# Aceinna/gnss-ins-sim

Hardware: AMD Instinct MI355X
Metric: Monte-Carlo IMU samples integrated/sec (higher is better)
Workload: dtype f64

## Files before the change

### gnss-ins-sim_amd/csrc/ginsim_api.hip

```cpp
#include <hip/hip_runtime.h>
#include <chrono>

#include <cmath>
#include <cstdarg>
#include <cstdio>
#include <cstring>
#include <string>
#include <vector>

#include "ginsim.h"
#include "ginsim_oallan.h"
#include "ginsim_psd.h"
#include "ginsim_lpsd.h"
#include "ginsim_csd.h"
#include "ginsim_loose_all.h"
#include "ginsim_loose_all_cons.h"
#include "allan.hpp"
#include "oallan.hpp"
#include "psd.hpp"
#include "lpsd.hpp"
#include "csd.hpp"
#include "comm.hpp"
#include "launch.hpp"
#include "placed.hpp"

namespace ginsim {

static thread_local std::string g_err;

void set_error(const char* fmt, ...) {
    char buf[512];
    va_list ap;
    va_start(ap, fmt);
    vsnprintf(buf, sizeof(buf), fmt, ap);
    va_end(ap);
    g_err = buf;
}

}

using namespace ginsim;

struct ginsim_ctx {
    int device;
    hipStream_t stream;
    hipEvent_t ev0, ev1;
    std::vector<hipEvent_t> pool;
    void* ws[4] = {nullptr, nullptr, nullptr, nullptr};
    size_t ws_bytes[4] = {0, 0, 0, 0};
    double* allan_host = nullptr;
    size_t allan_host_doubles = 0;
    int max_grid_y = 65535;
    ginsim::Comm* comm = nullptr;
    double* comm_recv = nullptr;
    ginsim_stats* comm_host = nullptr;
    hipEvent_t comm_ev[8] = {};
    bool comm_pending[8] = {};
    ginsim_stats* stat_slots = nullptr;
    hipEvent_t stat_ev[8] = {};
    bool stat_pending[8] = {};
    unsigned long long* selftest = nullptr;
};

static hipError_t scratch(ginsim_ctx* c, int slot, size_t bytes, void** out) {
    if (c->ws_bytes[slot] < bytes) {
        if (c->ws[slot]) {
            hipError_t e = hipStreamSynchronize(c->stream);
            if (e != hipSuccess) return e;
            e = hipFree(c->ws[slot]);
            if (e != hipSuccess) return e;
            c->ws[slot] = nullptr;
            c->ws_bytes[slot] = 0;
        }
        const size_t want = bytes + bytes / 4 + 4096;
        hipError_t e = hipMalloc(&c->ws[slot], want);
        if (e != hipSuccess) return e;
        c->ws_bytes[slot] = want;
    }
    *out = c->ws[slot];
    return hipSuccess;
}

#define HIP_TRY(expr)                                                                         \
    do {                                                                                      \
        hipError_t e_ = (expr);                                                               \
        if (e_ != hipSuccess) {                                                               \
            set_error("%s failed: %s (%s:%d)", #expr, hipGetErrorString(e_), __FILE__, __LINE__); \
            if (e_ == hipErrorOutOfMemory) { (void)hipGetLastError(); return GINSIM_ERR_NOMEM; } \
            return GINSIM_ERR_HIP;                                                            \
        }                                                                                     \
    } while (0)

#define REQUIRE(cond, ...)            \
    do {                              \
        if (!(cond)) {                \
            set_error(__VA_ARGS__);   \
            return GINSIM_ERR_ARG;    \
        }                             \
    } while (0)

struct DevBuf {
    void* p = nullptr;
    ~DevBuf() { if (p) (void)hipFree(p); }
    hipError_t alloc(size_t bytes) { return hipMalloc(&p, bytes ? bytes : 8); }
    template <class T> T* as() const { return reinterpret_cast<T*>(p); }
};

template <class Launch>
static int gather_run(const char* who, ginsim_ctx* c, const void* series, int32_t ncomp, int64_t n, int64_t runs, const int64_t* run_ids,
                      int32_t nsel, double* host_out, Launch launch) {
    REQUIRE(c && series && run_ids && host_out, "%s: NULL argument", who);
    REQUIRE(ncomp >= 1 && n >= 1 && runs >= 1 && nsel >= 1, "%s: bad sizes", who);
    for (int i = 0; i < nsel; ++i)
        REQUIRE(run_ids[i] >= 0 && run_ids[i] < runs, "%s: run id %lld out of range", who, (long long)run_ids[i]);
    HIP_TRY(hipSetDevice(c->device));
    DevBuf ids, out;
    const size_t out_bytes = sizeof(double) * (size_t)nsel * n * ncomp;
    HIP_TRY(ids.alloc(sizeof(int64_t) * nsel));
    HIP_TRY(out.alloc(out_bytes));
    HIP_TRY(hipMemcpyAsync(ids.p, run_ids, sizeof(int64_t) * nsel, hipMemcpyHostToDevice, c->stream));
    HIP_TRY(launch(ids.as<int64_t>(), out.as<double>()));
    HIP_TRY(hipMemcpyAsync(host_out, out.p, out_bytes, hipMemcpyDeviceToHost, c->stream));
    HIP_TRY(hipStreamSynchronize(c->stream));
    return GINSIM_OK;
}

template <class Launch>
static int traj_run(ginsim_ctx* c, TrajView v, size_t body, double* host_out, size_t out_bytes, Launch launch) {
    HIP_TRY(hipSetDevice(c->device));
    void* ws = nullptr;
    HIP_TRY(scratch(c, 2, body + sizeof(int64_t) * (size_t)v.m, &ws));
    if (v.samples) {
        int64_t* d_samples = reinterpret_cast<int64_t*>(reinterpret_cast<char*>(ws) + body);
        HIP_TRY(hipMemcpyAsync(d_samples, v.samples, sizeof(int64_t) * (size_t)v.m, hipMemcpyHostToDevice, c->stream));
        v.samples = d_samples;
    }
    HIP_TRY(launch(v, ws));
    if (out_bytes) HIP_TRY(hipMemcpyAsync(host_out, ws, out_bytes, hipMemcpyDeviceToHost, c->stream));
    HIP_TRY(hipStreamSynchronize(c->stream));
    return GINSIM_OK;
}

struct AllanStep { int k; int mode; };
struct AllanPlan {
    std::vector<int64_t> mult;
    int levels = 0;
    std::vector<AllanLevel> lvs;
    AllanFold fold;
    int64_t records = 0;
    std::vector<AllanStep> steps;
    std::vector<int32_t> mode, chunks_per_block, nparts;
};

static int allan_factors(int64_t n, double fs, std::vector<int64_t>& mult, int64_t* mmax_out) {
    const double ts = 1.0 / fs;
    const int64_t mmax = *mmax_out = (int64_t)floor((double)n / 9.0);
    if ((double)mmax * ts < 1.0) return 0;
    const int decades = (int)ceil(log10((double)mmax));
    double scale = 0.1;
    for (int i = 0; i < decades; ++i) {
        scale *= 10;
        for (int j = 1; j < 10; ++j) {
            const int64_t m = (int64_t)(j * scale);
            if (m > mmax) break;
            mult.push_back(m);
        }
    }
    return decades;
}

static int allan_plan(const double* x, int64_t n, int32_t nseries, int64_t series_stride, double fs, AllanPlan& P) {
    REQUIRE(n >= 1 && nseries >= 1 && series_stride >= n && fs > 0, "allan: bad sizes");
    int64_t mmax = 0;
    const int decades = allan_factors(n, fs, P.mult, &mmax);
    if ((double)mmax * (1.0 / fs) < 1.0) return GINSIM_OK;
    const int levels = P.levels = decades;
    std::vector<AllanLevel>& lvs = P.lvs;
    lvs.resize(levels);
    AllanFold& fold = P.fold;
    fold.nlevels = 0;
    fold.fused_level = -1;
    fold.pad = 0;
    for (int j = 0; j < 9; ++j) fold.fused_nb[j] = 0;
    int64_t& records = P.records;
    std::vector<AllanStep>& steps = P.steps;
    P.mode.assign(levels, 4);
    P.chunks_per_block.assign(levels, 1);
    P.nparts.assign(levels, 1);
    {
        int64_t n_in = n, stride_in = series_stride, pow10 = 1;
        for (int k = 0; k < levels; ++k) {
            AllanLevel& lv = lvs[k];
            lv.n_in = n_in;
            lv.n_out = (k + 1 < levels) ? n_in / 10 : 0;
            lv.in_stride = stride_in;
            lv.out_stride = lv.n_out;
            for (int j = 1; j <= 9; ++j) lv.nb[j - 1] = (j * pow10 <= mmax) ? n / (j * pow10) : 0;
            lv.nchunks = allan_chunks(n_in);
            lv.chunks_per_block = allan_chunks_per_block((int64_t)lv.nchunks * nseries);
            stride_in = lv.n_out;
            n_in = lv.n_out;
            pow10 *= 10;
        }
        int k = 0;
        if (levels >= 2 && lvs[0].n_in > allan_chunk_entries() && allan_fuse_applies(x, lvs[0], lvs[1])) {
            const int parts = allan_fuse_parts(lvs[0]);
            fold.nparts[0] = parts;
            fold.offset[0] = records;
            records += (int64_t)parts * nseries;
            fold.nparts[1] = parts;
            fold.offset[1] = records;
// ... 703 lines not shown
        REQUIRE(!L.scale_truth || L.scale, "loose_all_cons_run: scale_truth without a scale block");
    }
    if (L.cons && L.cons->cons_m == 0) L.cons = nullptr;
    if (L.mag && L.mag->mag_every == 0) L.mag = nullptr;
    if (L.still && L.still->still_mask == 0) L.still = nullptr;
    L.all_cons = who == LOOSE_ALL_CONS && L.cons != nullptr;
    L.all = (who == LOOSE_ALL || who == LOOSE_ALL_CONS) && (L.mag != nullptr) + (L.scale != nullptr) + (L.still != nullptr) >= 2;
    if (L.name) {
        L.name[0] = 0;
        (void)launch_loose(L);
        return GINSIM_OK;
    }
    HIP_TRY(hipSetDevice(c->device));
    const ginsim_loose_params* p = L.b;
    const size_t sb = sizeof(int64_t) * (size_t)p->m, vb = (sizeof(int32_t) * (size_t)p->m + 7) / 8 * 8;
    const size_t cb = L.cons ? sizeof(int64_t) * (size_t)L.cons->cons_m : 0;
    if (sb + cb > 0) {
        void* ws = nullptr;
        HIP_TRY(scratch(c, 3, sb + vb + cb, &ws));
        if (p->m > 0) {
            int64_t* d_stamp = reinterpret_cast<int64_t*>(ws);
            HIP_TRY(hipMemcpyAsync(d_stamp, p->gps_stamp, sb, hipMemcpyHostToDevice, c->stream));
            L.stamp = d_stamp;
            if (p->gps_visible) {
                int32_t* d_vis = reinterpret_cast<int32_t*>(reinterpret_cast<char*>(ws) + sb);
                HIP_TRY(hipMemcpyAsync(d_vis, p->gps_visible, sizeof(int32_t) * (size_t)p->m, hipMemcpyHostToDevice, c->stream));
                L.visible = d_vis;
            }
        }
        if (cb > 0) {
            int64_t* d_cons = reinterpret_cast<int64_t*>(reinterpret_cast<char*>(ws) + sb + vb);
            HIP_TRY(hipMemcpyAsync(d_cons, L.cons->cons_sample, cb, hipMemcpyHostToDevice, c->stream));
            L.samples = d_cons;
        }
    }
    L.stream = c->stream;
    HIP_TRY(launch_loose(L));
    return GINSIM_OK;
}

int ginsim_loose_kernel_name(const ginsim_mc_params* mc, const ginsim_loose_params* p, char* buf, size_t cap) {
    REQUIRE(buf && cap > 0, "loose_kernel_name: bad arguments");
    return loose_entry(LOOSE_PLAIN, nullptr, LooseLaunch{mc, p, nullptr, nullptr, nullptr, nullptr, buf, cap});
}

int ginsim_loose_run(ginsim_ctx* c, const ginsim_mc_params* mc, const ginsim_loose_params* p) {
    REQUIRE(c, "loose_run: NULL argument");
    return loose_entry(LOOSE_PLAIN, c, LooseLaunch{mc, p});
}

int ginsim_loose_cons_kernel_name(const ginsim_mc_params* mc, const ginsim_loose_params* p, const ginsim_loose_cons_params* cons,
                                  char* buf, size_t cap) {
    REQUIRE(buf && cap > 0, "loose_cons_kernel_name: bad arguments");
    return loose_entry(LOOSE_CONS, nullptr, LooseLaunch{mc, p, cons, nullptr, nullptr, nullptr, buf, cap});
}

int ginsim_loose_cons_run(ginsim_ctx* c, const ginsim_mc_params* mc, const ginsim_loose_params* p, const ginsim_loose_cons_params* cons) {
    REQUIRE(c, "loose_cons_run: NULL argument");
    return loose_entry(LOOSE_CONS, c, LooseLaunch{mc, p, cons});
}

int ginsim_loose_mag_kernel_name(const ginsim_mc_params* mc, const ginsim_loose_params* p, const ginsim_loose_mag_params* mag,
                                 char* buf, size_t cap) {
    REQUIRE(buf && cap > 0, "loose_mag_kernel_name: bad arguments");
    return loose_entry(LOOSE_MAG, nullptr, LooseLaunch{mc, p, nullptr, mag, nullptr, nullptr, buf, cap});
}

int ginsim_loose_mag_run(ginsim_ctx* c, const ginsim_mc_params* mc, const ginsim_loose_params* p, const ginsim_loose_mag_params* mag) {
    REQUIRE(c, "loose_mag_run: NULL argument");
    return loose_entry(LOOSE_MAG, c, LooseLaunch{mc, p, nullptr, mag});
}

int ginsim_loose_scale_kernel_name(const ginsim_mc_params* mc, const ginsim_loose_params* p, const ginsim_loose_scale_params* scale,
                                   char* buf, size_t cap) {
    REQUIRE(buf && cap > 0, "loose_scale_kernel_name: bad arguments");
    return loose_entry(LOOSE_SCALE, nullptr, LooseLaunch{mc, p, nullptr, nullptr, scale, nullptr, buf, cap});
}

int ginsim_loose_scale_run(ginsim_ctx* c, const ginsim_mc_params* mc, const ginsim_loose_params* p, const ginsim_loose_scale_params* scale) {
    REQUIRE(c, "loose_scale_run: NULL argument");
    return loose_entry(LOOSE_SCALE, c, LooseLaunch{mc, p, nullptr, nullptr, scale});
}

int ginsim_loose_still_kernel_name(const ginsim_mc_params* mc, const ginsim_loose_params* p, const ginsim_loose_still_params* still,
                                   char* buf, size_t cap) {
    REQUIRE(buf && cap > 0, "loose_still_kernel_name: bad arguments");
    return loose_entry(LOOSE_STILL, nullptr, LooseLaunch{mc, p, nullptr, nullptr, nullptr, still, buf, cap});
}

int ginsim_loose_still_run(ginsim_ctx* c, const ginsim_mc_params* mc, const ginsim_loose_params* p, const ginsim_loose_still_params* still) {
    REQUIRE(c, "loose_still_run: NULL argument");
    return loose_entry(LOOSE_STILL, c, LooseLaunch{mc, p, nullptr, nullptr, nullptr, still});
}

int ginsim_loose_all_kernel_name(const ginsim_mc_params* mc, const ginsim_loose_params* p, const ginsim_loose_mag_params* mag,
                                 const ginsim_loose_scale_params* scale, const ginsim_loose_still_params* still, char* buf, size_t cap) {
    REQUIRE(buf && cap > 0, "loose_all_kernel_name: bad arguments");
    return loose_entry(LOOSE_ALL, nullptr, LooseLaunch{mc, p, nullptr, mag, scale, still, buf, cap});
}

int ginsim_loose_all_run(ginsim_ctx* c, const ginsim_mc_params* mc, const ginsim_loose_params* p, const ginsim_loose_mag_params* mag,
                         const ginsim_loose_scale_params* scale, const ginsim_loose_still_params* still) {
    REQUIRE(c, "loose_all_run: NULL argument");
    return loose_entry(LOOSE_ALL, c, LooseLaunch{mc, p, nullptr, mag, scale, still});
}

int ginsim_loose_all_cons_kernel_name(const ginsim_mc_params* mc, const ginsim_loose_params* p, const ginsim_loose_mag_params* mag,
                                      const ginsim_loose_scale_params* scale, const ginsim_loose_still_params* still,
                                      const ginsim_loose_cons_params* cons, const double* scale_truth, char* buf, size_t cap) {
    REQUIRE(buf && cap > 0, "loose_all_cons_kernel_name: bad arguments");
    LooseLaunch L{mc, p, cons, mag, scale, still, buf, cap};
    L.scale_truth = scale_truth;
    return loose_entry(LOOSE_ALL_CONS, nullptr, L);
}

int ginsim_loose_all_cons_run(ginsim_ctx* c, const ginsim_mc_params* mc, const ginsim_loose_params* p, const ginsim_loose_mag_params* mag,
                              const ginsim_loose_scale_params* scale, const ginsim_loose_still_params* still,
                              const ginsim_loose_cons_params* cons, const double* scale_truth) {
    REQUIRE(c, "loose_all_cons_run: NULL argument");
    LooseLaunch L{mc, p, cons, mag, scale, still};
    L.scale_truth = scale_truth;
    return loose_entry(LOOSE_ALL_CONS, c, L);
}

int ginsim_aux_sensors(ginsim_ctx* c, const ginsim_aux_params* p) {
    REQUIRE(c && p, "aux_sensors: NULL argument");
    REQUIRE(p->runs >= 1 && p->n >= 0 && p->m >= 0, "aux_sensors: bad sizes");
    REQUIRE(!p->out_gps || p->ref_gps, "aux_sensors: ref_gps missing");
    REQUIRE(!p->out_mag || p->ref_mag, "aux_sensors: ref_mag missing");
    REQUIRE(p->n <= 0xFFFFFFFFll && p->m <= 0xFFFFFFFFll, "aux_sensors: sample index exceeds the RNG counter");
    REQUIRE((double)p->n * (double)p->runs < 5.0e11 && (double)p->m * (double)p->runs < 5.0e11, "aux_sensors: too many elements");
    HIP_TRY(hipSetDevice(c->device));
    HIP_TRY(launch_aux(*p, c->stream));
    return GINSIM_OK;
}

int ginsim_magcal_run(ginsim_ctx* c, const ginsim_magcal_params* p) {
    REQUIRE(c && p, "magcal_run: NULL argument");
    REQUIRE(p->runs >= 1, "magcal_run: runs=%lld must be >= 1", (long long)p->runs);
    REQUIRE(p->n >= 1 && p->n <= 0xFFFFFFFFll, "magcal_run: n must lie in 1 .. the 32-bit sample counter of the RNG");
    REQUIRE(p->runs <= (int64_t)0x7FFFFFFF * 64, "magcal_run: too many runs for one launch");
    REQUIRE(p->in_mag || p->ref_mag, "magcal_run: neither ref_mag (generated form) nor in_mag (given form)");
    REQUIRE(p->out_si && p->out_hi, "magcal_run: out_si / out_hi missing");
    for (int a = 0; a < 3; ++a) {
        const long long s0 = (long long)p->seg[2 * a], s1 = (long long)p->seg[2 * a + 1];
        REQUIRE(s0 >= 0 && s1 <= (long long)p->n, "magcal_run: range %c [%lld, %lld) is outside [0, %lld]", "xyz"[a], s0, s1, (long long)p->n);
        REQUIRE(s0 < s1, "magcal_run: range %c [%lld, %lld) is empty", "xyz"[a], s0, s1);
    }
    HIP_TRY(hipSetDevice(c->device));
    HIP_TRY(launch_magcal(*p, c->stream));
    return GINSIM_OK;
}

int ginsim_end_stats(ginsim_ctx* c, const double* end_err, int64_t runs, ginsim_stats* host_out) {
    REQUIRE(c && end_err && host_out && runs >= 1, "end_stats: bad arguments");
    HIP_TRY(hipSetDevice(c->device));
    void* ws = nullptr;
    HIP_TRY(scratch(c, 0, stats_scratch_bytes(runs), &ws));
    HIP_TRY(launch_end_stats(end_err, runs, ws, c->stream));
    const char* res = reinterpret_cast<char*>(ws) + stats_scratch_bytes(runs) - sizeof(ginsim_stats);
    HIP_TRY(hipMemcpyAsync(host_out, res, sizeof(ginsim_stats), hipMemcpyDeviceToHost, c->stream));
    HIP_TRY(hipStreamSynchronize(c->stream));
    return GINSIM_OK;
}

int ginsim_end_stats_begin(ginsim_ctx* c, const double* end_err, int64_t runs, int32_t slot) {
    REQUIRE(c && end_err && runs >= 1 && slot >= 0 && slot < 8, "end_stats_begin: bad arguments");
    REQUIRE(!c->stat_pending[slot], "end_stats_begin: slot %d is still pending (call ginsim_end_stats_finish first)", slot);
    HIP_TRY(hipSetDevice(c->device));
    if (!c->stat_slots) HIP_TRY(hipHostMalloc(reinterpret_cast<void**>(&c->stat_slots), 8 * sizeof(ginsim_stats), hipHostMallocDefault));
    if (!c->stat_ev[slot]) HIP_TRY(hipEventCreateWithFlags(&c->stat_ev[slot], hipEventDisableTiming));
    void* ws = nullptr;
    HIP_TRY(scratch(c, 0, stats_scratch_bytes(runs), &ws));
    HIP_TRY(launch_end_stats(end_err, runs, ws, c->stream));
    const char* res = reinterpret_cast<char*>(ws) + stats_scratch_bytes(runs) - sizeof(ginsim_stats);
    HIP_TRY(hipMemcpyAsync(&c->stat_slots[slot], res, sizeof(ginsim_stats), hipMemcpyDeviceToHost, c->stream));
    HIP_TRY(hipEventRecord(c->stat_ev[slot], c->stream));
    c->stat_pending[slot] = true;
    return GINSIM_OK;
}

int ginsim_end_stats_finish(ginsim_ctx* c, int32_t slot, ginsim_stats* host_out) {
    REQUIRE(c && host_out && slot >= 0 && slot < 8, "end_stats_finish: bad arguments");
    REQUIRE(c->stat_pending[slot], "end_stats_finish: nothing was begun in slot %d", slot);
    HIP_TRY(hipEventSynchronize(c->stat_ev[slot]));
    *host_out = c->stat_slots[slot];
    c->stat_pending[slot] = false;
    return GINSIM_OK;
}

int ginsim_comm_unique_id(unsigned char* id) {
    REQUIRE(id, "comm_unique_id: NULL output");
    const char* err = comm_unique_id(id);
    if (err) { set_error("comm_unique_id: %s", err); return GINSIM_ERR_HIP; }
    return GINSIM_OK;
}

int ginsim_comm_init(ginsim_ctx* c, int32_t nranks, int32_t rank, const unsigned char* id) {
    REQUIRE(c && id && nranks >= 1 && rank >= 0 && rank < nranks, "comm_init: bad arguments");
    REQUIRE(!c->comm, "comm_init: this context already has a communicator");
    HIP_TRY(hipSetDevice(c->device));
    const size_t bytes = sizeof(ginsim_stats) * 8 * (size_t)nranks;
    hipError_t e = hipMalloc(reinterpret_cast<void**>(&c->comm_recv), bytes);
    if (e == hipSuccess) e = hipHostMalloc(reinterpret_cast<void**>(&c->comm_host), bytes, hipHostMallocDefault);
    const char* err = e == hipSuccess ? comm_create(nranks, rank, id, &c->comm) : nullptr;
    if (e != hipSuccess || err) {
        if (c->comm_recv) { (void)hipFree(c->comm_recv); c->comm_recv = nullptr; }
        if (c->comm_host) { (void)hipHostFree(c->comm_host); c->comm_host = nullptr; }
        c->comm = nullptr;
        if (err) set_error("comm_init: %s", err);
        else set_error("comm_init: %s", hipGetErrorString(e));
        return GINSIM_ERR_HIP;
    }
    return GINSIM_OK;
}

int ginsim_comm_probe(void) {
    const char* err = comm_probe();
    if (err) { set_error("comm_probe: %s", err); return GINSIM_ERR_HIP; }
    return GINSIM_OK;
}

__global__ void first_xcc_kernel(uint32_t* out) {
    if (threadIdx.x == 0) out[0] = __builtin_amdgcn_s_getreg((31 << 11) | 20) & 0xf;
}

int ginsim_stream_first_xcc(ginsim_ctx* c, int32_t* xcc) {
    REQUIRE(c && xcc, "stream_first_xcc: NULL argument");
    HIP_TRY(hipSetDevice(c->device));
    void* ws = nullptr;
    HIP_TRY(scratch(c, 2, 64, &ws));
    hipLaunchKernelGGL(first_xcc_kernel, dim3(1), dim3(64), 0, c->stream, reinterpret_cast<uint32_t*>(ws));
    HIP_TRY(hipGetLastError());
    uint32_t v = 0;
    HIP_TRY(hipMemcpyAsync(&v, ws, sizeof v, hipMemcpyDeviceToHost, c->stream));
    HIP_TRY(hipStreamSynchronize(c->stream));
    *xcc = (int32_t)v;
    return GINSIM_OK;
}

int ginsim_vib_psd_series(ginsim_ctx* c, const double* amp, int64_t period, int64_t runs, uint64_t run_offset, uint64_t seed,
                          int32_t sensor, int32_t halve_per_run, double* out) {
    REQUIRE(c && amp && out, "vib_psd_series: NULL argument");
    REQUIRE(period >= 2 && period <= 16384 && period % 2 == 0, "vib_psd_series: period %lld must be even, 2 .. 16384 (time_series_from_psd.py:36-43)",
            (long long)period);
    REQUIRE(runs >= 1 && runs <= (int64_t)0x7FFFFFFF * 64, "vib_psd_series: runs=%lld out of range", (long long)runs);
    REQUIRE(sensor == 0 || sensor == 1, "vib_psd_series: sensor must be 0 (accelerometer) or 1 (gyroscope)");
    REQUIRE(halve_per_run == 0 || halve_per_run == 1, "vib_psd_series: halve_per_run must be 0 or 1");
    for (int64_t k = 0; k < 3 * (period / 2 + 1); ++k)
        REQUIRE(std::isfinite(amp[k]) && amp[k] >= 0.0, "vib_psd_series: amplitude %lld is negative or not finite", (long long)k);
    HIP_TRY(hipSetDevice(c->device));
    void* ws = nullptr;
    HIP_TRY(scratch(c, 3, vib_psd_scratch_bytes(period, runs), &ws));
    return launch_vib_psd(c->device, c->stream, amp, period, runs, run_offset, seed, sensor, halve_per_run, ws, out);
}

int ginsim_comm_query(ginsim_ctx* c, int32_t* nranks, int32_t* rank, int32_t* device) {
    REQUIRE(c && nranks && rank && device, "comm_query: bad arguments");
    REQUIRE(c->comm, "comm_query: no communicator (ginsim_comm_init)");
    int n = -1, r = -1, d = -1;
    const char* err = comm_query(c->comm, &n, &r, &d);
    if (err) { set_error("comm_query: %s", err); return GINSIM_ERR_HIP; }
    *nranks = n; *rank = r; *device = d;
    return GINSIM_OK;
}

int ginsim_comm_destroy(ginsim_ctx* c) {
    REQUIRE(c, "comm_destroy: NULL context");
    if (!c->comm) return GINSIM_OK;
    HIP_TRY(hipSetDevice(c->device));
    HIP_TRY(hipStreamSynchronize(c->stream));
    comm_destroy(c->comm);
    c->comm = nullptr;
    if (c->comm_recv) { (void)hipFree(c->comm_recv); c->comm_recv = nullptr; }
    if (c->comm_host) { (void)hipHostFree(c->comm_host); c->comm_host = nullptr; }
    for (bool& p : c->comm_pending) p = false;
    return GINSIM_OK;
}

int ginsim_end_stats_all_begin(ginsim_ctx* c, const double* end_err, int64_t runs, int32_t slot) {
    REQUIRE(c && runs >= 0 && (runs == 0 || end_err) && slot >= 0 && slot < 8, "end_stats_all_begin: bad arguments");
    REQUIRE(c->comm && c->comm_recv && c->comm_host, "end_stats_all_begin: no communicator (ginsim_comm_init)");
    REQUIRE(!c->comm_pending[slot], "end_stats_all_begin: slot %d is still pending (call ginsim_end_stats_all_finish first)", slot);
    HIP_TRY(hipSetDevice(c->device));
    if (!c->comm_ev[slot]) HIP_TRY(hipEventCreateWithFlags(&c->comm_ev[slot], hipEventDisableTiming));
    const int nranks = comm_nranks(c->comm);
    void* ws = nullptr;
    const size_t wb = stats_scratch_bytes(runs > 0 ? runs : 1);
    HIP_TRY(scratch(c, 0, wb, &ws));
    double* rec = reinterpret_cast<double*>(reinterpret_cast<char*>(ws) + wb - sizeof(ginsim_stats));
    if (runs > 0) HIP_TRY(launch_end_stats(end_err, runs, ws, c->stream));
    else HIP_TRY(hipMemsetAsync(rec, 0, sizeof(ginsim_stats), c->stream));
    double* recv = c->comm_recv + (size_t)slot * nranks * (sizeof(ginsim_stats) / sizeof(double));
    const char* err = comm_allgather_f64(c->comm, rec, recv, sizeof(ginsim_stats) / sizeof(double), c->stream);
    if (err) { set_error("end_stats_all_begin: %s", err); return GINSIM_ERR_HIP; }
    HIP_TRY(hipMemcpyAsync(c->comm_host + (size_t)slot * nranks, recv, sizeof(ginsim_stats) * nranks, hipMemcpyDeviceToHost, c->stream));
    HIP_TRY(hipEventRecord(c->comm_ev[slot], c->stream));
    c->comm_pending[slot] = true;
    return GINSIM_OK;
}

int ginsim_end_stats_all_finish(ginsim_ctx* c, int32_t slot, ginsim_stats* merged) {
    REQUIRE(c && merged && slot >= 0 && slot < 8, "end_stats_all_finish: bad arguments");
    REQUIRE(c->comm && c->comm_pending[slot], "end_stats_all_finish: nothing was begun in slot %d", slot);
    HIP_TRY(hipEventSynchronize(c->comm_ev[slot]));
    c->comm_pending[slot] = false;
    const int nranks = comm_nranks(c->comm);
    std::vector<ginsim_stats> parts;
    for (int r = 0; r < nranks; ++r) {
        const ginsim_stats& p = c->comm_host[(size_t)slot * nranks + r];
        if (p.count > 0) parts.push_back(p);
    }
    memset(merged, 0, sizeof(*merged));
    if (!parts.empty()) stats_merge_host(parts.data(), (int)parts.size(), merged);
    return GINSIM_OK;
}

static int traj_stats_run(ginsim_ctx* c, const TrajView& v, int64_t first_sample, int32_t pos_ned, double* proc_out, ginsim_stats* end_out) {
    HIP_TRY(hipSetDevice(c->device));
    void* ws = nullptr;
    const size_t bytes = sizeof(double) * 27 * (size_t)v.runs;
    HIP_TRY(scratch(c, 2, bytes, &ws));
    double* rec = reinterpret_cast<double*>(ws);
    HIP_TRY(launch_process_stats(v, proc_out ? first_sample : v.n - 1, pos_ned, proc_out ? 1 : 0, rec, c->stream));
    if (!proc_out) return ginsim_end_stats(c, rec + (size_t)9 * v.runs, v.runs, end_out);
    HIP_TRY(hipMemcpyAsync(proc_out, ws, bytes, hipMemcpyDeviceToHost, c->stream));
    HIP_TRY(hipStreamSynchronize(c->stream));
    return GINSIM_OK;
}

int ginsim_process_stats(ginsim_ctx* c, const double* traj, const double* ref, int64_t n, int64_t runs, int64_t first_sample,
                         int32_t pos_ned, double* host_out) {
    REQUIRE(c && traj && ref && host_out, "process_stats: NULL argument");
    REQUIRE(n >= 1 && runs >= 1 && first_sample >= 0 && first_sample < n, "process_stats: bad sizes");
    return traj_stats_run(c, TrajView{traj, 0, ref, n, runs, nullptr, 0, {nullptr, 0, 0}}, first_sample, pos_ned, host_out, nullptr);
}

int ginsim_end_stats_from_traj(ginsim_ctx* c, const double* traj, const double* ref, int64_t n, int64_t runs, int32_t pos_ned,
                               ginsim_stats* host_out) {
    REQUIRE(c && traj && ref && host_out && n >= 1 && runs >= 1, "end_stats_from_traj: bad arguments");
    return traj_stats_run(c, TrajView{traj, 0, ref, n, runs, nullptr, 0, {nullptr, 0, 0}}, 0, pos_ned, nullptr, host_out);
}

int ginsim_process_stats_f32(ginsim_ctx* c, const float* traj, const double* ref, int64_t n, int64_t runs, int64_t first_sample,
                             int32_t pos_ned, const double* origin, int32_t n_ini, uint64_t ini_first, double* host_out) {
    REQUIRE(c && traj && ref && origin && host_out, "process_stats_f32: NULL argument");
    REQUIRE(n >= 1 && runs >= 1 && first_sample >= 0 && first_sample < n && n_ini >= 1, "process_stats_f32: bad sizes");
    return traj_stats_run(c, TrajView{traj, 1, ref, n, runs, nullptr, 0, {origin, n_ini, ini_first}}, first_sample, pos_ned, host_out, nullptr);
}

int ginsim_end_stats_from_traj_f32(ginsim_ctx* c, const float* traj, const double* ref, int64_t n, int64_t runs, int32_t pos_ned,
                                   const double* origin, int32_t n_ini, uint64_t ini_first, ginsim_stats* host_out) {
    REQUIRE(c && traj && ref && origin && host_out && n >= 1 && runs >= 1 && n_ini >= 1, "end_stats_from_traj_f32: bad arguments");
    return traj_stats_run(c, TrajView{traj, 1, ref, n, runs, nullptr, 0, {origin, n_ini, ini_first}}, 0, pos_ned, nullptr, host_out);
}

static int check_curve_args(const char* who, const void* c, const TrajView& v, const void* host_out) {
    const int64_t n = v.n, m = v.m;
    REQUIRE(c && v.traj && v.ref && host_out, "%s: NULL argument", who);
    REQUIRE(n >= 1 && v.runs >= 1, "%s: n=%lld runs=%lld must be >= 1", who, (long long)n, (long long)v.runs);
    REQUIRE(m >= 1, "%s: m=%lld samples (at least one is needed)", who, (long long)m);
    REQUIRE(v.samples || m == n, "%s: samples == NULL means every sample, so m must be n (m=%lld, n=%lld)", who, (long long)m, (long long)n);
    REQUIRE(m <= 0x7FFFFFFFll, "%s: too many samples for one call", who);
    if (v.samples)
        for (int64_t i = 0; i < m; ++i)
            REQUIRE(v.samples[i] >= 0 && v.samples[i] < n, "%s: sample %lld (entry %lld) is outside [0, %lld)", who, (long long)v.samples[i],
                    (long long)i, (long long)n);
    return GINSIM_OK;
}

static int check_which(const char* who, int32_t which) {
    REQUIRE(which == 0 || which == 1, "%s: which=%d is neither 0 (position) nor 1 (velocity)", who, (int)which);
    return GINSIM_OK;
}

static int check_origin(const char* who, const TrajView& v) {
    REQUIRE(!v.f32 || (v.org.table && v.org.n_ini >= 1), "%s: the origin table of the displacement series is missing", who);
    return GINSIM_OK;
}

static int curve_entry(const char* who, ginsim_ctx* c, const TrajView& v, int32_t pos_ned, double* host_out) {
    int rc = check_curve_args(who, c, v, host_out);
    if (!rc) rc = check_origin(who, v);
    if (rc) return rc;
    return traj_run(c, v, error_curve_scratch_bytes(v), host_out, sizeof(double) * 36 * (size_t)v.m,
                    [&](const TrajView& d, void* ws) { return launch_error_curve(d, pos_ned, ws, c->stream); });
}

int ginsim_error_curve(ginsim_ctx* c, const double* traj, const double* ref, int64_t n, int64_t runs, const int64_t* samples, int64_t m,
                       int32_t pos_ned, double* host_out) {
    return curve_entry("error_curve", c, TrajView{traj, 0, ref, n, runs, samples, m, {nullptr, 0, 0}}, pos_ned, host_out);
}

int ginsim_error_curve_f32(ginsim_ctx* c, const float* traj, const double* ref, int64_t n, int64_t runs, const int64_t* samples,
                           int64_t m, int32_t pos_ned, const double* origin, int32_t n_ini, uint64_t ini_first, double* host_out) {
    return curve_entry("error_curve_f32", c, TrajView{traj, 1, ref, n, runs, samples, m, {origin, n_ini, ini_first}}, pos_ned, host_out);
}

int ginsim_curve_merge(const double* parts, int32_t nparts, int64_t m, double* out) {
    REQUIRE(parts && out && nparts >= 1 && m >= 1, "curve_merge: bad arguments");
    curve_merge_host(parts, nparts, m, out);
    return GINSIM_OK;
}

static int keys_entry(const char* who, ginsim_ctx* c, const TrajView& v, int32_t which, int32_t pos_ned, double* keys, int64_t row_stride,
                      int64_t col0) {
    int rc = check_curve_args(who, c, v, keys);
    if (!rc) rc = check_which(who, which);
    if (rc) return rc;
    REQUIRE(col0 >= 0, "%s: col0=%lld is negative", who, (long long)col0);
    REQUIRE(row_stride >= col0 + v.runs, "%s: row_stride=%lld is shorter than col0 + runs = %lld + %lld", who, (long long)row_stride,
            (long long)col0, (long long)v.runs);
    rc = check_origin(who, v);
    if (rc) return rc;
    return traj_run(c, v, 0, nullptr, 0, [&](const TrajView& d, void*) {
        return launch_radial_keys(d, which, pos_ned, keys, row_stride, col0, c->stream);
    });
}

int ginsim_radial_keys(ginsim_ctx* c, const double* traj, const double* ref, int64_t n, int64_t runs, const int64_t* samples, int64_t m,
                       int32_t which, int32_t pos_ned, double* keys, int64_t row_stride, int64_t col0) {
    return keys_entry("radial_keys", c, TrajView{traj, 0, ref, n, runs, samples, m, {nullptr, 0, 0}}, which, pos_ned, keys, row_stride, col0);
}

int ginsim_radial_keys_f32(ginsim_ctx* c, const float* traj, const double* ref, int64_t n, int64_t runs, const int64_t* samples,
                           int64_t m, int32_t which, int32_t pos_ned, const double* origin, int32_t n_ini, uint64_t ini_first,
                           double* keys, int64_t row_stride, int64_t col0) {
    return keys_entry("radial_keys_f32", c, TrajView{traj, 1, ref, n, runs, samples, m, {origin, n_ini, ini_first}}, which, pos_ned, keys,
                      row_stride, col0);
}

int ginsim_quantile_rows(ginsim_ctx* c, const double* keys, int64_t rows, int64_t len, int64_t row_stride, const double* probs,
                         int32_t q, double* host_out, double* host_count) {
    REQUIRE(c && keys && probs && host_out && host_count, "quantile_rows: NULL argument");
    REQUIRE(rows >= 1 && len >= 1, "quantile_rows: rows=%lld len=%lld must be >= 1", (long long)rows, (long long)len);
    REQUIRE(rows <= 0x7FFFFFFFll && len <= 0x7FFFFFFFll, "quantile_rows: too many rows or keys for one call");
    REQUIRE(row_stride >= len, "quantile_rows: row_stride=%lld is shorter than len=%lld", (long long)row_stride, (long long)len);
    REQUIRE(q >= 1 && q <= GINSIM_QUANTILE_MAX_PROBS, "quantile_rows: q=%d probabilities (1..%d at once)", (int)q,
            GINSIM_QUANTILE_MAX_PROBS);
    for (int i = 0; i < q; ++i)
        REQUIRE(std::isfinite(probs[i]) && probs[i] > 0.0 && probs[i] <= 1.0, "quantile_rows: probability %g (entry %d) is not in (0, 1]",
                probs[i], i);
    HIP_TRY(hipSetDevice(c->device));
    const size_t res = sizeof(double) * (size_t)rows * ((size_t)q + 1);
// ... 658 lines not shown
```

### gnss-ins-sim_amd/csrc/launch.hpp

```cpp
#pragma once
#include <hip/hip_runtime.h>
#include <stdint.h>
#include <stdlib.h>
#include "ginsim.h"

namespace ginsim {

void set_error(const char* fmt, ...);

hipError_t launch_mc(const ginsim_mc_params& p, hipStream_t stream, char* name, size_t cap, double* proc_about);
int mc_variant(const ginsim_mc_params& p);

hipError_t launch_mc_f32(const ginsim_mc_params& p, float* truth32, hipStream_t stream, char* name, size_t cap);
size_t mc_f32_truth_bytes(const ginsim_mc_params& p);
int mc_variant_f32(const ginsim_mc_params& p);

bool series_path_applies(const ginsim_mc_params& p);
int series_pass_b(const ginsim_mc_params& p);
int64_t series_chunks(const ginsim_mc_params& p, int32_t* L_out);
hipError_t launch_series(const ginsim_mc_params& p, double* carry, hipStream_t stream);

hipError_t launch_incl(const ginsim_mc_params& p, const ginsim_incl_params& b, hipStream_t stream, char* name, size_t cap);
int incl_variant(const ginsim_mc_params& p);

struct LooseLaunch {
    const ginsim_mc_params* mc;
    const ginsim_loose_params* b;
    const ginsim_loose_cons_params* cons;
    const ginsim_loose_mag_params* mag;
    const ginsim_loose_scale_params* scale;
    const ginsim_loose_still_params* still;
    char* name; size_t cap;
    const int64_t* stamp;
    const int32_t* visible;
    const int64_t* samples;
    hipStream_t stream;
    bool all;
    bool all_cons;
    const double* scale_truth;
};

hipError_t launch_loose_plain(const LooseLaunch& L);
hipError_t launch_loose_aided(const LooseLaunch& L);
hipError_t launch_loose_cons(const LooseLaunch& L);
hipError_t launch_loose_mag(const LooseLaunch& L);
hipError_t launch_loose_scale(const LooseLaunch& L);
hipError_t launch_loose_still(const LooseLaunch& L);
hipError_t launch_loose_all(const LooseLaunch& L);
hipError_t launch_loose_all16(const LooseLaunch& L);
hipError_t launch_loose_all_cons(const LooseLaunch& L);
hipError_t launch_loose_all_cons16(const LooseLaunch& L);
hipError_t launch_cons_final(const ginsim_loose_cons_params& c, int64_t waves, hipStream_t stream);
int loose_variant(const ginsim_mc_params& p);

hipError_t launch_aux(const ginsim_aux_params& p, hipStream_t s);

hipError_t launch_magcal(const ginsim_magcal_params& p, hipStream_t s);

size_t vib_psd_scratch_bytes(int64_t period, int64_t runs);
int launch_vib_psd(int device, hipStream_t stream, const double* amp, int64_t period, int64_t runs, uint64_t run_offset, uint64_t seed,
                   int sensor, int halve, void* scratch, double* out);
void vib_psd_drop_plans(hipStream_t stream);

hipError_t launch_rng_probe(uint64_t seed, uint64_t run, uint32_t stream, int64_t count, double* z0, double* z1,
                            uint32_t* words, hipStream_t stream_h);
hipError_t launch_normal_transform(const uint32_t* words, int64_t count, double* z0, double* z1, hipStream_t s);

hipError_t launch_aos_to_soa(const double* src, double* dst, int64_t R, int64_t n, int C, hipStream_t s);
hipError_t launch_runs_to_series(const double* in, double* out, int C, int64_t n, int64_t R, hipStream_t s);
hipError_t launch_gather_runs(const double* series, int C, int64_t n, int64_t runs, const int64_t* ids, int nsel,
                              double* out, hipStream_t s);
hipError_t launch_gather_series(const double* series, int C, int64_t n, const int64_t* ids, int nsel, double* out, hipStream_t s);
hipError_t launch_gather_runs_f32(const float* series, int C, int64_t n, int64_t runs, const int64_t* ids, int nsel,
                                  double* out, hipStream_t s);

hipError_t launch_pattern_fill(void* p, uint64_t words, uint32_t tag, hipStream_t s);
hipError_t launch_pattern_check(const void* p, uint64_t words, uint32_t tag, unsigned long long* out, hipStream_t s);
hipError_t launch_digest(const void* p, uint64_t words, unsigned long long* out, hipStream_t s);

struct ProcOrigin {
    const double* table;
    int64_t n_ini;
    uint64_t ini_first;
};

struct TrajView {
    const void* traj;
    int f32;
    const double* ref;
    int64_t n, runs;
    const int64_t* samples;
    int64_t m;
    ProcOrigin org;
};

size_t stats_scratch_bytes(int64_t runs);
int stats_blocks(int64_t runs);
hipError_t launch_end_stats(const double* end_err, int64_t runs, void* scratch, hipStream_t s);
void stats_merge_host(const ginsim_stats* parts, int nparts, ginsim_stats* out);
hipError_t launch_process_stats(const TrajView& v, int64_t j0, int pos_ned, int run_major, double* out, hipStream_t s);

size_t error_curve_scratch_bytes(const TrajView& v);
hipError_t launch_error_curve(const TrajView& v, int pos_ned, void* scratch, hipStream_t s);
void curve_merge_host(const double* parts, int nparts, int64_t m, double* out);

hipError_t launch_radial_keys(const TrajView& v, int which, int pos_ned, double* keys, int64_t row_stride, int64_t col0, hipStream_t s);
hipError_t launch_quantile_rows(const double* keys, int64_t rows, int64_t len, int64_t row_stride, const double* probs, int q,
                                double* out, double* count, hipStream_t s);

size_t error_cov_scratch_bytes(const TrajView& v);
hipError_t launch_error_cov(const TrajView& v, int which, int pos_ned, void* scratch, hipStream_t s);
void cov_merge_host(const double* parts, int nparts, int64_t m, double* out);

inline int split_policy() {
    static const int v = [] { const char* e = getenv("GINSIM_SPLIT"); return e ? atoi(e) : -1; }();
    return v;
}

inline bool any_vibration(const ginsim_mc_params& p) { return p.vib_accel.type != GINSIM_VIB_NONE || p.vib_gyro.type != GINSIM_VIB_NONE; }
inline bool any_psd_vibration(const ginsim_mc_params& p) { return p.vib_accel.type == GINSIM_VIB_PSD || p.vib_gyro.type == GINSIM_VIB_PSD; }

inline bool any_white_drift(const ginsim_mc_params& p) {
    bool f = false;
    for (int k = 0; k < 3; ++k)
        f = f || p.accel.white_drift[k] || p.gyro.white_drift[k] || p.accel.bias[k] != 0.0 || p.gyro.bias[k] != 0.0;
    return f;
}

}
```

### gnss-ins-sim_amd/csrc/stats.hip

```cpp
#include <hip/hip_runtime.h>
#include "ginsim.h"
#include "fastmath.hpp"
#include "ins_math.hpp"
#include "traj_error.hpp"

namespace ginsim {

constexpr int kStatBlock = 256;

__device__ __forceinline__ double shift_of(const double* x) {
    const double k = x[0];
    return __builtin_isfinite(k) ? k : 0.0;
}

__global__ void __launch_bounds__(kStatBlock) stats_partial_kernel(const double* __restrict__ e, int64_t runs,
                                                                   Mom* __restrict__ partial) {
    const int comp = blockIdx.y;
    const double* x = e + (int64_t)comp * runs;
    const double k = shift_of(x);
    Mom m{0.0, 0.0, 0.0, 0.0};
    for (int64_t r = (int64_t)blockIdx.x * kStatBlock + threadIdx.x; r < runs; r += (int64_t)gridDim.x * kStatBlock) {
        const double v = x[r] - k;
        m.n += 1.0;
        if (__builtin_isfinite(v) && __builtin_isfinite(m.mean)) {
            const double d = v - m.mean;
            m.mean += d / m.n;
            m.m2 += d * (v - m.mean);
        } else {
            m.mean += v;
            m.m2 = __builtin_nan("");
        }
        m.mx = nan_max(fabs(x[r]), m.mx);
    }
#pragma unroll
    for (int mask = 32; mask >= 1; mask >>= 1) m = merge(m, shfl_xor(m, mask));
    __shared__ Mom wave_part[kStatBlock / 64];
    if ((threadIdx.x & 63) == 0) wave_part[threadIdx.x >> 6] = m;
    __syncthreads();
    if (threadIdx.x == 0) {
        Mom t = wave_part[0];
        for (int w = 1; w < kStatBlock / 64; ++w) t = merge(t, wave_part[w]);
        partial[comp * gridDim.x + blockIdx.x] = t;
    }
}

__global__ void stats_final_kernel(const Mom* __restrict__ partial, int blocks, const double* __restrict__ e, int64_t runs,
                                   ginsim_stats* __restrict__ out) {
    const int c = blockIdx.x;
    Mom t{0.0, 0.0, 0.0, 0.0};
    for (int b = threadIdx.x; b < blocks; b += 64) t = merge(t, partial[c * blocks + b]);
#pragma unroll
    for (int mask = 32; mask >= 1; mask >>= 1) t = merge(t, shfl_xor(t, mask));
    if (threadIdx.x == 0) {
        if (c == 0) out->count = t.n;
        out->mean[c] = shift_of(e + (int64_t)c * runs) + t.mean;
        out->m2[c] = t.m2;
        out->maxabs[c] = t.mx;
    }
}

constexpr int kSeg = 4;

template <typename T>
__global__ void __launch_bounds__(64 * kSeg) process_stats_kernel(const T* __restrict__ traj, const double* __restrict__ ref,
                                                                 int64_t n, int64_t runs, int64_t j0, int pos_ned,
                                                                 int run_major, double* __restrict__ out, const ProcOrigin org) {
    __shared__ Mom part[kSeg][9][64];
    const int lane = threadIdx.x & 63, seg = threadIdx.x >> 6;
    const int64_t r = (int64_t)blockIdx.x * 64 + lane;
    const bool active = r < runs;
    const int64_t plane = n * runs;
    const uniform_ref truth = (uniform_ref)(uintptr_t)ref;
    const int64_t len = n - j0, per = (len + kSeg - 1) / kSeg;
    const int64_t jb = j0 + seg * per, je = (jb + per < n) ? jb + per : n;
    double mean[9], m2[9], mx[9];
#pragma unroll
    for (int c = 0; c < 9; ++c) { mean[c] = 0.0; m2[c] = 0.0; mx[c] = 0.0; }
    double cnt = 0.0;
    double o3[3] = {0.0, 0.0, 0.0};
    if (org.table && active) run_origin(org, r, o3);
    auto error = [&](int64_t j, double (&e)[9]) {
        double x[9], t[9];
#pragma unroll
        for (int c = 0; c < 9; ++c) { x[c] = (double)traj[c * plane + j * runs + r]; t[c] = truth[9 * j + c]; }
        x[3] += o3[0]; x[4] += o3[1]; x[5] += o3[2];
        sample_error(x, t, pos_ned, e);
    };
    if (active) {
        for (int64_t j = jb; j < je; ++j) {
            double e[9];
            error(j, e);
            cnt += 1.0;
            const double icnt = rcp_nr(cnt);
#pragma unroll
            for (int c = 0; c < 9; ++c) {
                const double d = e[c] - mean[c];
                mean[c] = __builtin_fma(d, icnt, mean[c]);
                m2[c] = __builtin_fma(d, e[c] - mean[c], m2[c]);
                mx[c] = nan_max(fabs(e[c]), mx[c]);
            }
        }
        bool bad = false;
#pragma unroll
        for (int c = 0; c < 9; ++c) bad |= !__builtin_isfinite(mx[c]);
        if (bad) {
            double sum[9];
#pragma unroll
            for (int c = 0; c < 9; ++c) sum[c] = 0.0;
            for (int64_t j = jb; j < je; ++j) {
                double e[9];
                error(j, e);
#pragma unroll
                for (int c = 0; c < 9; ++c) sum[c] += e[c];
            }
#pragma unroll
            for (int c = 0; c < 9; ++c)
                if (!__builtin_isfinite(mx[c])) { mean[c] = sum[c] / cnt; m2[c] = __builtin_nan(""); }
        }
    }
#pragma unroll
    for (int c = 0; c < 9; ++c) part[seg][c][lane] = Mom{cnt, mean[c], m2[c], mx[c]};
    __syncthreads();
    if (seg == 0 && active) {
#pragma unroll
        for (int c = 0; c < 9; ++c) {
            Mom t = part[0][c][lane];
#pragma unroll
            for (int k = 1; k < kSeg; ++k) t = merge(t, part[k][c][lane]);
            const double sd = t.n > 0.0 ? sqrt(t.m2 / t.n) : 0.0;
            if (run_major) {
                out[(r * 3 + 0) * 9 + c] = t.mx;
                out[(r * 3 + 1) * 9 + c] = t.mean;
                out[(r * 3 + 2) * 9 + c] = sd;
            } else {
                out[(0 * 9 + c) * runs + r] = t.mx;
                out[(1 * 9 + c) * runs + r] = t.mean;
                out[(2 * 9 + c) * runs + r] = sd;
            }
        }
    }
}

template <typename T>
static hipError_t launch_proc(const TrajView& v, int64_t j0, int pos_ned, int run_major, double* out, hipStream_t s) {
    hipLaunchKernelGGL((process_stats_kernel<T>), dim3((unsigned)((v.runs + 63) / 64)), dim3(64 * kSeg), 0, s,
                       static_cast<const T*>(v.traj), v.ref, v.n, v.runs, j0, pos_ned, run_major, out, v.org);
    return hipGetLastError();
}

hipError_t launch_process_stats(const TrajView& v, int64_t j0, int pos_ned, int run_major, double* out, hipStream_t s) {
    return v.f32 ? launch_proc<float>(v, j0, pos_ned, run_major, out, s) : launch_proc<double>(v, j0, pos_ned, run_major, out, s);
}

int stats_blocks(int64_t runs) {
    int64_t b = (runs + kStatBlock - 1) / kStatBlock;
    return (int)(b < 1 ? 1 : (b > 256 ? 256 : b));
}

size_t stats_scratch_bytes(int64_t runs) { return sizeof(Mom) * 9 * (size_t)stats_blocks(runs) + sizeof(ginsim_stats); }

hipError_t launch_end_stats(const double* end_err, int64_t runs, void* scratch, hipStream_t s) {
    const int blocks = stats_blocks(runs);
    Mom* partial = reinterpret_cast<Mom*>(scratch);
    ginsim_stats* out = reinterpret_cast<ginsim_stats*>(partial + 9 * blocks);
    hipLaunchKernelGGL(stats_partial_kernel, dim3(blocks, 9), dim3(kStatBlock), 0, s, end_err, runs, partial);
    hipLaunchKernelGGL(stats_final_kernel, dim3(9), dim3(64), 0, s, partial, blocks, end_err, runs, out);
    return hipGetLastError();
}

void stats_merge_host(const ginsim_stats* parts, int nparts, ginsim_stats* out) {
    for (int c = 0; c < 9; ++c) {
        Mom t{0.0, 0.0, 0.0, 0.0};
        for (int k = 0; k < nparts; ++k)
            t = merge(t, Mom{parts[k].count, parts[k].mean[c], parts[k].m2[c], parts[k].maxabs[c]});
        out->count = t.n;
        out->mean[c] = t.mean;
        out->m2[c] = t.m2;
        out->maxabs[c] = t.mx;
    }
}

}
```

Before: 54.64 billion.

## Write end-stats directly to mapped host memory and fast-path equal-count wave merges

The final stats kernel now stores its result record straight into pinned, device-mapped host memory using system-scope stores. This removes the separate device-to-host memcpy in the blocking and async end-stats paths. The wave-level Welford merge also gains a fast path for lanes that all hold the same count, which avoids the general merge arithmetic. The costs are uncached PCIe/XGMI writes from the kernel and a slightly larger pinned allocation holding nine slots.

```diff
diff --git a/gnss-ins-sim_amd/csrc/ginsim_api.hip b/gnss-ins-sim_amd/csrc/ginsim_api.hip
--- a/gnss-ins-sim_amd/csrc/ginsim_api.hip
+++ b/gnss-ins-sim_amd/csrc/ginsim_api.hip
@@ -57,6 +57,7 @@
     hipEvent_t comm_ev[8] = {};
     bool comm_pending[8] = {};
     ginsim_stats* stat_slots = nullptr;
+    ginsim_stats* stat_slots_dev = nullptr;
     hipEvent_t stat_ev[8] = {};
     bool stat_pending[8] = {};
     unsigned long long* selftest = nullptr;
@@ -1066,15 +1067,30 @@
     return GINSIM_OK;
 }
 
+static hipError_t stat_slot(ginsim_ctx* c, int slot, ginsim_stats** dev) {
+    if (!c->stat_slots) {
+        hipError_t e = hipHostMalloc(reinterpret_cast<void**>(&c->stat_slots), 9 * sizeof(ginsim_stats), hipHostMallocDefault);
+        if (e == hipSuccess) e = hipHostGetDevicePointer(reinterpret_cast<void**>(&c->stat_slots_dev), c->stat_slots, 0);
+        if (e != hipSuccess) {
+            if (c->stat_slots) (void)hipHostFree(c->stat_slots);
+            c->stat_slots = nullptr;
+            return e;
+        }
+    }
+    *dev = c->stat_slots_dev + slot;
+    return hipSuccess;
+}
+
 int ginsim_end_stats(ginsim_ctx* c, const double* end_err, int64_t runs, ginsim_stats* host_out) {
     REQUIRE(c && end_err && host_out && runs >= 1, "end_stats: bad arguments");
     HIP_TRY(hipSetDevice(c->device));
+    ginsim_stats* rec = nullptr;
+    HIP_TRY(stat_slot(c, 8, &rec));
     void* ws = nullptr;
     HIP_TRY(scratch(c, 0, stats_scratch_bytes(runs), &ws));
-    HIP_TRY(launch_end_stats(end_err, runs, ws, c->stream));
-    const char* res = reinterpret_cast<char*>(ws) + stats_scratch_bytes(runs) - sizeof(ginsim_stats);
-    HIP_TRY(hipMemcpyAsync(host_out, res, sizeof(ginsim_stats), hipMemcpyDeviceToHost, c->stream));
-    HIP_TRY(hipStreamSynchronize(c->stream));
+    HIP_TRY(launch_end_stats(end_err, runs, ws, rec, c->stream));
+    HIP_TRY(hipStreamSynchronize(c->stream));
+    *host_out = c->stat_slots[8];
     return GINSIM_OK;
 }
 
@@ -1082,13 +1098,12 @@
     REQUIRE(c && end_err && runs >= 1 && slot >= 0 && slot < 8, "end_stats_begin: bad arguments");
     REQUIRE(!c->stat_pending[slot], "end_stats_begin: slot %d is still pending (call ginsim_end_stats_finish first)", slot);
     HIP_TRY(hipSetDevice(c->device));
-    if (!c->stat_slots) HIP_TRY(hipHostMalloc(reinterpret_cast<void**>(&c->stat_slots), 8 * sizeof(ginsim_stats), hipHostMallocDefault));
+    ginsim_stats* rec = nullptr;
+    HIP_TRY(stat_slot(c, slot, &rec));
     if (!c->stat_ev[slot]) HIP_TRY(hipEventCreateWithFlags(&c->stat_ev[slot], hipEventDisableTiming));
     void* ws = nullptr;
     HIP_TRY(scratch(c, 0, stats_scratch_bytes(runs), &ws));
-    HIP_TRY(launch_end_stats(end_err, runs, ws, c->stream));
-    const char* res = reinterpret_cast<char*>(ws) + stats_scratch_bytes(runs) - sizeof(ginsim_stats);
-    HIP_TRY(hipMemcpyAsync(&c->stat_slots[slot], res, sizeof(ginsim_stats), hipMemcpyDeviceToHost, c->stream));
+    HIP_TRY(launch_end_stats(end_err, runs, ws, rec, c->stream));
     HIP_TRY(hipEventRecord(c->stat_ev[slot], c->stream));
     c->stat_pending[slot] = true;
     return GINSIM_OK;
@@ -1202,8 +1217,9 @@
     void* ws = nullptr;
     const size_t wb = stats_scratch_bytes(runs > 0 ? runs : 1);
     HIP_TRY(scratch(c, 0, wb, &ws));
-    double* rec = reinterpret_cast<double*>(reinterpret_cast<char*>(ws) + wb - sizeof(ginsim_stats));
-    if (runs > 0) HIP_TRY(launch_end_stats(end_err, runs, ws, c->stream));
+    ginsim_stats* dst = stats_scratch_record(ws, runs > 0 ? runs : 1);
+    double* rec = reinterpret_cast<double*>(dst);
+    if (runs > 0) HIP_TRY(launch_end_stats(end_err, runs, ws, dst, c->stream));
     else HIP_TRY(hipMemsetAsync(rec, 0, sizeof(ginsim_stats), c->stream));
     double* recv = c->comm_recv + (size_t)slot * nranks * (sizeof(ginsim_stats) / sizeof(double));
     const char* err = comm_allgather_f64(c->comm, rec, recv, sizeof(ginsim_stats) / sizeof(double), c->stream);
diff --git a/gnss-ins-sim_amd/csrc/launch.hpp b/gnss-ins-sim_amd/csrc/launch.hpp
--- a/gnss-ins-sim_amd/csrc/launch.hpp
+++ b/gnss-ins-sim_amd/csrc/launch.hpp
@@ -96,7 +96,8 @@
 
 size_t stats_scratch_bytes(int64_t runs);
 int stats_blocks(int64_t runs);
-hipError_t launch_end_stats(const double* end_err, int64_t runs, void* scratch, hipStream_t s);
+ginsim_stats* stats_scratch_record(void* scratch, int64_t runs);
+hipError_t launch_end_stats(const double* end_err, int64_t runs, void* scratch, ginsim_stats* out, hipStream_t s);
 void stats_merge_host(const ginsim_stats* parts, int nparts, ginsim_stats* out);
 hipError_t launch_process_stats(const TrajView& v, int64_t j0, int pos_ned, int run_major, double* out, hipStream_t s);
 
diff --git a/gnss-ins-sim_amd/csrc/stats.hip b/gnss-ins-sim_amd/csrc/stats.hip
--- a/gnss-ins-sim_amd/csrc/stats.hip
+++ b/gnss-ins-sim_amd/csrc/stats.hip
@@ -11,6 +11,32 @@
 __device__ __forceinline__ double shift_of(const double* x) {
     const double k = x[0];
     return __builtin_isfinite(k) ? k : 0.0;
+}
+
+__device__ __forceinline__ double first_lane(double v) {
+    const unsigned long long u = __builtin_bit_cast(unsigned long long, v);
+    const unsigned lo = __builtin_amdgcn_readfirstlane((unsigned)u), hi = __builtin_amdgcn_readfirstlane((unsigned)(u >> 32));
+    return __builtin_bit_cast(double, ((unsigned long long)hi << 32) | lo);
+}
+
+__device__ __forceinline__ Mom merge_xor(const Mom& a, int mask) {
+    const double n0 = first_lane(a.n);
+    if (__all(a.n == n0) && n0 > 0.0 && n0 < 67108864.0) {
+        Mom o;
+        const double bmean = __shfl_xor(a.mean, mask, 64), bm2 = __shfl_xor(a.m2, mask, 64), bmx = __shfl_xor(a.mx, mask, 64);
+        o.n = a.n + a.n;
+        if (__builtin_isfinite(a.mean) && __builtin_isfinite(bmean)) {
+            const double d = bmean - a.mean;
+            o.mean = a.mean + d * 0.5;
+            o.m2 = a.m2 + bm2 + d * d * (0.5 * a.n);
+        } else {
+            o.mean = a.mean + bmean;
+            o.m2 = __builtin_nan("");
+        }
+        o.mx = nan_max(a.mx, bmx);
+        return o;
+    }
+    return merge(a, shfl_xor(a, mask));
 }
 
 __global__ void __launch_bounds__(kStatBlock) stats_partial_kernel(const double* __restrict__ e, int64_t runs,
@@ -33,7 +59,7 @@
         m.mx = nan_max(fabs(x[r]), m.mx);
     }
 #pragma unroll
-    for (int mask = 32; mask >= 1; mask >>= 1) m = merge(m, shfl_xor(m, mask));
+    for (int mask = 32; mask >= 1; mask >>= 1) m = merge_xor(m, mask);
     __shared__ Mom wave_part[kStatBlock / 64];
     if ((threadIdx.x & 63) == 0) wave_part[threadIdx.x >> 6] = m;
     __syncthreads();
@@ -44,18 +70,22 @@
     }
 }
 
+__device__ __forceinline__ void store_sys(double* p, double v) {
+    __hip_atomic_store(p, v, __ATOMIC_RELAXED, __HIP_MEMORY_SCOPE_SYSTEM);
+}
+
 __global__ void stats_final_kernel(const Mom* __restrict__ partial, int blocks, const double* __restrict__ e, int64_t runs,
                                    ginsim_stats* __restrict__ out) {
     const int c = blockIdx.x;
     Mom t{0.0, 0.0, 0.0, 0.0};
     for (int b = threadIdx.x; b < blocks; b += 64) t = merge(t, partial[c * blocks + b]);
 #pragma unroll
-    for (int mask = 32; mask >= 1; mask >>= 1) t = merge(t, shfl_xor(t, mask));
+    for (int mask = 32; mask >= 1; mask >>= 1) t = merge_xor(t, mask);
     if (threadIdx.x == 0) {
-        if (c == 0) out->count = t.n;
-        out->mean[c] = shift_of(e + (int64_t)c * runs) + t.mean;
-        out->m2[c] = t.m2;
-        out->maxabs[c] = t.mx;
+        if (c == 0) store_sys(&out->count, t.n);
+        store_sys(&out->mean[c], shift_of(e + (int64_t)c * runs) + t.mean);
+        store_sys(&out->m2[c], t.m2);
+        store_sys(&out->maxabs[c], t.mx);
     }
 }
 
@@ -159,10 +189,13 @@
 
 size_t stats_scratch_bytes(int64_t runs) { return sizeof(Mom) * 9 * (size_t)stats_blocks(runs) + sizeof(ginsim_stats); }
 
-hipError_t launch_end_stats(const double* end_err, int64_t runs, void* scratch, hipStream_t s) {
+ginsim_stats* stats_scratch_record(void* scratch, int64_t runs) {
+    return reinterpret_cast<ginsim_stats*>(reinterpret_cast<Mom*>(scratch) + 9 * stats_blocks(runs));
+}
+
+hipError_t launch_end_stats(const double* end_err, int64_t runs, void* scratch, ginsim_stats* out, hipStream_t s) {
     const int blocks = stats_blocks(runs);
     Mom* partial = reinterpret_cast<Mom*>(scratch);
-    ginsim_stats* out = reinterpret_cast<ginsim_stats*>(partial + 9 * blocks);
     hipLaunchKernelGGL(stats_partial_kernel, dim3(blocks, 9), dim3(kStatBlock), 0, s, end_err, runs, partial);
     hipLaunchKernelGGL(stats_final_kernel, dim3(9), dim3(64), 0, s, partial, blocks, end_err, runs, out);
     return hipGetLastError();
```

Result: no change. 54.82 billion (median of 2 runs) (+0.3%).
